# cvxopt/smcp

Measured on AMD Instinct MI355X. Metric: Newton KKT solves/sec, higher is better.
Workload: dtype f64; 1 GPU; synth50k nested block-arrow SDP n=50000, 8073 cliques, m=100; kktsolver=chol, n=50000, cliques=8073, m=100, blkval_doubles=2493568, update_doubles=10689536, parallelism=single

## Files before the change

### smcp_amd/build.py

```python
import os
import shutil
import subprocess
import sys

HERE = os.path.dirname(os.path.abspath(__file__))
CSRC = os.path.join(HERE, "csrc")
LIB = os.path.join(HERE, "libsmcp_amd.so")
SOURCES = ["capi.hip", "symbolic.cpp"]
DEPS = ["front_large.hip", "front_mfma.hip", "capi.hip", "kkt.hip", "kkt_qr.hip", "front_generic.hip", "front_mrc.hip", "front_edm.hip", "front_psd.hip", "front_downfam.hip", "front_upfam.hip", "wgblas.hpp", "context.hpp", "symbolic.cpp",
        "symbolic.hpp", "../../include/smcp_amd.h"]


def _stale():
    if not os.path.exists(LIB):
        return True
    t = os.path.getmtime(LIB)
    for d in os.listdir(CSRC):
        if os.path.getmtime(os.path.join(CSRC, d)) > t:
            return True
    return os.path.getmtime(os.path.join(HERE, "..", "include", "smcp_amd.h")) > t


def build(force=False, verbose=True):
    if not force and not _stale():
        return LIB
    hipcc = shutil.which("hipcc") or "/opt/rocm/bin/hipcc"
    cmd = [hipcc, "--offload-arch=gfx950", "-O3", "-std=c++17", "-fPIC", "-shared",
           "-Wno-unused-result", "-Wno-unused-value", "-pthread", "-o", LIB] + [os.path.join(CSRC, s) for s in SOURCES]
    if os.environ.get("SMCP_STAMPS") == "1":
        cmd.insert(1, "-DSMCP_STAMPS")
    for flag in os.environ.get("SMCP_CXXFLAGS", "").split():
        cmd.insert(1, flag)
    if verbose:
        print(" ".join(cmd), file=sys.stderr)
    subprocess.check_call(cmd)
    return LIB


if __name__ == "__main__":
    build(force="--force" in sys.argv)
```

### smcp_amd/csrc/capi.hip

```cpp
#include <hip/hip_runtime.h>
#include <memory>
#include <unordered_map>

#include <algorithm>
#include <chrono>
#include <cstdio>
#include <cstring>
#include <map>
#include <new>
#include <atomic>
#include <thread>
#include <type_traits>
#include <vector>

#include "../../include/smcp_amd.h"
#include "context.hpp"
#include "switches.hpp"
#include "front_generic.hip"
#include "front_mfma.hip"
#include "front_large.hip"
#include "front_inv.hip"
#include "front_n16.hip"
#include "front_downfam.hip"
#include "front_fam.hip"
#include "front_upfam.hip"
#include "front_fam2.hip"
#include "front_lfsp.hip"
#include "front_leafgram.hip"
#include "front_famt.hip"
#include "front_flow.hip"
#include "front_mrc.hip"
#include "front_edm.hip"
#include "front_psd.hip"

using namespace smcp;

#define HIPCHK(x)                                                                        \
  do {                                                                                   \
    hipError_t e_ = (x);                                                                 \
    if (e_ != hipSuccess) {                                                              \
      fprintf(stderr, "smcp_amd: HIP error %s at %s:%d\n", hipGetErrorString(e_), __FILE__, __LINE__); \
      return SMCP_EHIP;                                                                  \
    }                                                                                    \
  } while (0)

namespace {

enum {
  KID_chol_level = 0, KID_llt_level, KID_pinv_level, KID_gather_level, KID_completion_all,
  KID_hess_up_level, KID_hess_down_level, KID_hess_down_inv_all, KID_hess_up_inv_level, KID_scale_an,
  KID_factor_yaa, KID_trsm_fwd_level, KID_trsm_bwd_level, KID_amap, KID_aadj, KID_scatter_constraints,
  KID_dense_potrf, KID_dense_potrs, KID_vec_axpby, KID_axpby, KID_reduce_cliques, KID_reduce_final,
  KID_hess_up_mfma, KID_hess_down_mfma, KID_chol_mfma, KID_pinv_mfma, KID_prep_lk,
  KID_hess_up_mfma_hbm, KID_hess_down_mfma_hbm, KID_chol_mfma_hbm, KID_pinv_mfma_hbm,
  KID_gram_partial, KID_gram_reduce, KID_hess_up_pad,
  KID_lf_assemble, KID_lf_clear_upd, KID_lf_up1, KID_lf_up2, KID_lf_up3, KID_lf_down1, KID_lf_down2, KID_lf_down3,
  KID_lf_pinv1, KID_lf_pinv2, KID_lf_diag, KID_lf_chol_panel, KID_lf_chol_trail, KID_lf_pack_upd,
  KID_lf_prep_s, KID_lf_prep_row, KID_lf_prep_k, KID_factor_yaa_lds,
  KID_factor_inverse, KID_hess_down_inv_mfma, KID_hess_down_inv_mfma_hbm, KID_hess_up_inv_mfma, KID_hess_up_inv_mfma_hbm,
  KID_completion_mfma, KID_completion_mfma_hbm, KID_lf_copy_an, KID_lf_ri_an, KID_lf_dinv1, KID_lf_dinv2,
  KID_lf_uinv1, KID_lf_uinv2, KID_lf_completion, KID_hess_up_n16, KID_llt_mfma, KID_llt_mfma_hbm, KID_lf_llt,
  KID_hess_up_fam, KID_qr_rmul, KID_qr_dots, KID_qr_comb, KID_qr_small, KID_fam2_prep, KID_mid_chol, KID_lf_diag_inv, KID_lfsp_up, KID_lfsp_prep, KID_leaf_gram, KID_leaf_tables, KID_fam_sparse, KID_gram_diag128, KID_lf_assemble_lds, KID_fam_terms, KID_famt_prep, KID_lf_assemble_lds_dyn, KID_lf_zsp, KID_fam_terms_grp, KID_lf_assemble_fz, KID_factor_inverse_lds, KID_chol_flow,
  KID_mrc_diag, KID_mrc_rank, KID_mrc_reduce, KID_mrc_factor, KID_cut_signs, KID_cut_weights,
  KID_edm_rank, KID_edm_reduce, KID_edm_factor, KID_edm_dense, KID_hess_down_fam, KID_hess_up_fam1,
  KID_psd_zero, KID_psd_scatter, KID_psd_solve, KID_psd_fill,
  KID_COUNT
};
const char* const KID_NAMES[KID_COUNT] = {
  "k_chol_level", "k_llt_level", "k_pinv_level", "k_gather_level", "k_completion_all",
  "k_hess_up_level", "k_hess_down_level", "k_hess_down_inv_all", "k_hess_up_inv_level", "k_scale_an",
  "k_factor_yaa", "k_trsm_fwd_level", "k_trsm_bwd_level", "k_amap", "k_aadj", "k_scatter_constraints",
  "k_dense_potrf", "k_dense_potrs", "k_vec_axpby", "k_axpby", "k_reduce_cliques", "k_reduce_final",
  "k_hess_up_mfma<true>", "k_hess_down_mfma<true>", "k_chol_mfma<true>", "k_pinv_mfma<true>", "k_prep_lk",
  "k_hess_up_mfma<false>", "k_hess_down_mfma<false>", "k_chol_mfma<false>", "k_pinv_mfma<false>",
  "k_gram_partial", "k_gram_reduce", "k_hess_up_pad",
  "k_lf_assemble", "k_lf_clear_upd", "k_lf_up1", "k_lf_up2", "k_lf_up3", "k_lf_down1", "k_lf_down2", "k_lf_down3",
  "k_lf_pinv1", "k_lf_pinv2", "k_lf_diag", "k_lf_chol_panel", "k_lf_chol_trail", "k_lf_pack_upd",
  "k_lf_prep_s", "k_lf_prep_row", "k_lf_prep_k", "k_factor_yaa_lds",
  "k_factor_inverse", "k_hess_down_inv_mfma<true>", "k_hess_down_inv_mfma<false>", "k_hess_up_inv_mfma<true>",
  "k_hess_up_inv_mfma<false>", "k_completion_mfma<true>", "k_completion_mfma<false>", "k_lf_copy_an", "k_lf_ri_an",
  "k_lf_dinv1", "k_lf_dinv2", "k_lf_uinv1", "k_lf_uinv2", "k_lf_completion", "k_hess_up_n16",
  "k_llt_mfma<true>", "k_llt_mfma<false>", "k_lf_llt", "k_hess_up_fam",
  "k_stack_trsm", "k_stack_dots", "k_stack_comb", "k_qr_small", "k_fam2_prep", "k_mid_chol", "k_lf_diag_inv", "k_lfsp_up", "k_lfsp_prep", "k_leaf_pairs", "k_leaf_tables", "k_fam_sparse", "k_gram_diag128", "k_lf_assemble_lds", "k_fam_terms", "k_famt_prep", "k_lf_assemble_lds_dyn", "k_lf_zsp", "k_fam_terms_grp", "k_lf_assemble_fz", "k_factor_inverse_lds", "k_chol_flow",
  "k_mrc_diag", "k_mrc_rank", "k_mrc_reduce", "k_mrc_factor", "k_cut_signs", "k_cut_weights",
  "k_edm_rank", "k_edm_reduce", "k_edm_factor", "k_edm_dense", "k_hess_down_fam", "k_hess_up_fam1",
  "k_psd_zero", "k_psd_scatter", "k_psd_solve", "k_psd_fill"};

inline void note_launch(csp_ctx* c, int kid) {
  const hipError_t e = hipGetLastError();
  if (e != hipSuccess && !c->launch_err) {
    c->launch_err = (int)e;
    fprintf(stderr, "smcp_amd: launch of %s failed: %s\n", (kid >= 0 && kid < KID_COUNT) ? KID_NAMES[kid] : "?", hipGetErrorString(e));
  }
}
inline hipError_t end_call(csp_ctx* c) {
  hipError_t e = hipGetLastError();
  if (e == hipSuccess && c->launch_err) e = c->launch_err > 0 ? (hipError_t)c->launch_err : hipErrorLaunchFailure;
  c->launch_err = 0;
  return e;
}

__global__ void k_race_spin(long long ticks) {
  const long long t0 = wall_clock64();
  for (int it = 0; it < (1 << 22) && wall_clock64() - t0 < ticks; ++it) __builtin_amdgcn_s_sleep(8);
}
struct RaceInject {
  std::atomic<uint64_t> state{0};
  std::atomic<int64_t> injected{0};
  std::atomic<int> max_us{200};
  std::atomic<int> drop_joins{0};
  bool on() const { return state.load(std::memory_order_relaxed) != 0; }
  void seed(uint64_t s) { state.store(s ? (s * 0x9E3779B97F4A7C15ull) | 1ull : 0ull); }
  uint64_t next() {
    uint64_t x = state.load(std::memory_order_relaxed);
    x ^= x << 13; x ^= x >> 7; x ^= x << 17;
    state.store(x | 1ull, std::memory_order_relaxed);
    return x;
  }
};
// ... 592 lines not shown
    csp_ctx::FlowPlanDev P;
    P.nwg = (int)optr.size() - 1;
    int64_t junk = 0;
    if (dev_upload(&P.own_ptr, optr, junk) || dev_upload(&P.own_tile, otile, junk)) { (void)hipGetLastError(); return false; }
    c->D.bytes += junk;
    it = c->flow_plans.emplace(plan_key, P).first;
  }
  FlowArgs f;
  f.A = A; f.ld = ld; f.n = n;
  f.dinv = dinv ? dinv : W.dinv;
  f.P = W.P; f.flags = W.flags;
  f.epoch = ++W.epoch;
  f.own_ptr = it->second.own_ptr; f.own_tile = it->second.own_tile;
  f.info = info; f.info_val = info_val;
  f.cl = fa ? fa->t.cl : nullptr; f.lev = fa ? fa->t.lev : nullptr; f.mode = mode; f.nsn1 = fa ? fa->t.nsn1 : 1;
  f.dbg = nullptr;
  f.p_stride = (int64_t)ntiles * 4096; f.dinv_stride = (int64_t)nt * 4096; f.flag_stride = ntiles + nt + 4;
  static int stamps = -1;
  if (stamps < 0) stamps = sw_on("SMCP_FLOW_STAMPS", 0);
  static long long* dbg = nullptr;
  if (stamps) { if (!dbg) (void)hipMalloc((void**)&dbg, sizeof(long long) * 16 * FLOW_MAXWG); f.dbg = dbg; }
  launch_lds(c, KID_chol_flow, k_chol_flow, dim3(it->second.nwg, cnt), dim3(256), FLOW_LDS_BYTES, st, f);
  if (stamps && dbg) {
    std::vector<long long> h((size_t)8 * it->second.nwg);
    (void)hipStreamSynchronize(st);
    (void)hipMemcpy(h.data(), dbg, h.size() * sizeof(long long), hipMemcpyDeviceToHost);
    for (int w = 0; w < std::min(it->second.nwg, 20); ++w)
      fprintf(stderr, "flow n %d wg %3d: idle %7.1f us (%lld)  update %7.1f us (%lld)  potrf %7.1f us (%lld)  panel %7.1f us (%lld)\n", n, w,
              h[8 * w] / 100.0, h[8 * w + 4], h[8 * w + 1] / 100.0, h[8 * w + 5], h[8 * w + 2] / 100.0, h[8 * w + 6], h[8 * w + 3] / 100.0, h[8 * w + 7]);
  }
  return true;
}

void lf_chol(csp_ctx* c, const MfmaArgs& a, int cnt, double* x, hipStream_t st) {
  dim3 blk(256);
  const int nfmax = a.nnmax + a.namax;
  lf_assemble(c, a, cnt, 1, x, 0, 0, st, true);
  if (use_mid(nfmax)) {
    launch_lds(c, KID_mid_chol, k_mid_chol, dim3(cnt), dim3(1024), mid_chol_lds(nfmax), st, a, x, (double*)nullptr, 0);
    return;
  }
  if (cnt == 1 && a.namax == 0 && flow_chol(c, st, x, 0, a.nnmax, nullptr, &a, 0, a.t.info, 0)) return;
  const int mtA = tiles64(a.namax);
  for (int jb = 0; jb < a.nnmax; jb += LB) {
    launch_lds(c, KID_lf_diag, k_lf_diag, dim3(cnt), diag_blk(), LF_DIAG_LDS, st, a, x, (double*)nullptr, 0, jb, 1);
    const int mrem = nfmax - jb - 1, ncr = std::max(0, a.nnmax - jb - 1);
    if (mrem > 0) launch(c, KID_lf_chol_panel, k_lf_chol_panel, dim3(umax1(tiles64(mrem)), cnt), blk, st, a, x, (double*)nullptr, 0, jb);
    const int mt = tiles64(mrem), nt = tiles64(ncr);
    const int ntask = nt * (nt + 1) / 2 + std::max(0, mt - nt) * nt + mtA * (mtA + 1) / 2;
    if (ntask > 0) launch(c, KID_lf_chol_trail, k_lf_chol_trail, dim3(umax1(ntask), cnt), blk, st, a, x, (double*)nullptr, 0, jb);
  }
  if (a.namax) launch(c, KID_lf_pack_upd, k_lf_pack_upd, dim3(umax1(std::min(64, (a.namax * a.namax + 255) / 256)), cnt), blk, st, a);
}
void lf_factor_yaa(csp_ctx* c, const MfmaArgs& a, int cnt, double* fac, hipStream_t st) {
  dim3 blk(256);
  if (use_mid(a.namax)) {
    launch_lds(c, KID_mid_chol, k_mid_chol, dim3(cnt), dim3(1024), mid_chol_lds(a.namax), st, a, (double*)nullptr, fac, 2);
    return;
  }
  if (flow_chol(c, st, fac, 0, a.namax, nullptr, &a, 2, a.t.info, 0, cnt)) return;
  for (int jb = 0; jb < a.namax; jb += LB) {
    launch_lds(c, KID_lf_diag, k_lf_diag, dim3(cnt), diag_blk(), LF_DIAG_LDS, st, a, (double*)nullptr, fac, 2, jb, 1);
    const int mrem = a.namax - jb - 1;
    if (mrem > 0) {
      launch(c, KID_lf_chol_panel, k_lf_chol_panel, dim3(umax1(tiles64(mrem)), cnt), blk, st, a, (double*)nullptr, fac, 2, jb);
      const int mt = tiles64(mrem);
      launch(c, KID_lf_chol_trail, k_lf_chol_trail, dim3(umax1(mt * (mt + 1) / 2), cnt), blk, st, a, (double*)nullptr, fac, 2, jb);
    }
  }
}
void lf_prep(csp_ctx* c, const MfmaArgs& a, int cnt, const double* L, hipStream_t st) {
  dim3 blk(256);
  static int hoist = -1;
  if (hoist < 0) { const char* e = sw_str("SMCP_MID"); hoist = (e && e[0] == '0') ? 0 : 1; }
  if (hoist) {
    launch_lds(c, KID_lf_diag_inv, k_lf_diag_inv, dim3(cnt, tiles64(a.nnmax)), blk, LF_DIAG_LDS, st, a, L, c->D.lk);
    static int rec = -1;
    if (rec < 0) { const char* e = sw_str("SMCP_TRTRI"); rec = (e && e[0] == '0') ? 0 : 1; }
    if (rec) {
      for (int b = LB; b < a.nnmax; b *= 2) {
        const int pairs = (a.nnmax + 2 * b - 1) / (2 * b), tpb = b / LB;
        for (int step = 0; step < 2; ++step)
          launch(c, KID_lf_prep_s, k_lf_trtri, dim3(umax1(pairs * tpb * tpb), cnt), blk, st, a, L, c->D.lk, b, step);
      }
    } else
    for (int ib = LB; ib < a.nnmax; ib += LB) {
      launch(c, KID_lf_prep_s, k_lf_prep_s, dim3(umax1(tiles64(ib)), cnt), blk, st, a, L, c->D.lk, ib, 0);
      launch(c, KID_lf_prep_row, k_lf_prep_row, dim3(umax1(tiles64(ib)), cnt), blk, st, a, L, c->D.lk, ib, 0, 1);
    }
  } else
  for (int ib = 0; ib < a.nnmax; ib += LB) {
    launch_lds(c, KID_lf_diag, k_lf_diag, dim3(cnt), diag_blk(), LF_DIAG_LDS, st, a, const_cast<double*>(L), (double*)nullptr, 1, ib, 0);
    if (ib > 0) launch(c, KID_lf_prep_s, k_lf_prep_s, dim3(umax1(tiles64(ib)), cnt), blk, st, a, L, c->D.lk, ib, 0);
    launch(c, KID_lf_prep_row, k_lf_prep_row, dim3(umax1(tiles64(ib) + 1), cnt), blk, st, a, L, c->D.lk, ib, 0, 0);
  }
  if (a.namax) launch(c, KID_lf_prep_k, k_lf_prep_k, dim3(umax1(tiles64(a.namax) * tiles64(a.nnmax)), cnt), blk, st, a, L, c->D.lk);
}

static size_t prep_lk_lds_bytes(int nnmax) { return nnmax > 16 ? (size_t)16 * 16 * 16 * sizeof(double) : 0; }
static int prep_lk_threads(int nnmax) { return nnmax > 16 ? NT : 128; }
__global__ void k_diag_fingerprint(const CliqueDesc* cl, int nsn, const double* x, unsigned long long* slot, int* bad, int check) {
  __shared__ unsigned long long part[256];
  unsigned long long s = 0;
  for (int k = blockIdx.x; k < nsn; k += gridDim.x) {
    const CliqueDesc d = cl[k];
    const int64_t len = (int64_t)(d.nn + d.na) * d.nn;
    for (int64_t e = threadIdx.x; e < len; e += blockDim.x)
      s += (unsigned long long)__double_as_longlong(x[d.blk + e]) * (2ull * (unsigned long long)(d.blk + e) + 1ull);
  }
  part[threadIdx.x] = s;
  __syncthreads();
  for (int o = 128; o > 0; o >>= 1) { if ((int)threadIdx.x < o) part[threadIdx.x] += part[threadIdx.x + o]; __syncthreads(); }
  if (threadIdx.x == 0) atomicAdd(slot + (check ? 4 : 0), part[0]);
  (void)bad;
}
__global__ void k_fingerprint_compare(unsigned long long* slots, int which, int* bad) {
  if (threadIdx.x == 0) { if (slots[which] != slots[which + 4]) *bad = 1 + which; slots[which + 4] = 0; }
}
static void fp_record(csp_ctx* c, int which, const double* x, hipStream_t st) {
  if (!c->verify_cache || !c->D.fp) return;
  (void)hipMemsetAsync(c->D.fp + which, 0, sizeof(unsigned long long), st);
  hipLaunchKernelGGL(k_diag_fingerprint, dim3(1024), dim3(256), 0, st, c->D.cl, (int)c->S.nsn, x, c->D.fp + which, c->D.fp_bad, 0);
}
static int fp_check(csp_ctx* c, int which, const double* x, hipStream_t st) {
  if (!c->verify_cache || !c->D.fp) return 0;
  hipLaunchKernelGGL(k_diag_fingerprint, dim3(1024), dim3(256), 0, st, c->D.cl, (int)c->S.nsn, x, c->D.fp + which, c->D.fp_bad, 1);
  hipLaunchKernelGGL(k_fingerprint_compare, dim3(1), dim3(64), 0, st, c->D.fp, which, c->D.fp_bad);
  int bad = 0;
  if (hipMemcpyAsync(&bad, c->D.fp_bad, sizeof(int), hipMemcpyDeviceToHost, st) != hipSuccess || hipStreamSynchronize(st) != hipSuccess) return SMCP_EHIP;
  if (bad) {
    (void)hipMemsetAsync(c->D.fp_bad, 0, sizeof(int), st);
    fprintf(stderr, "smcp_amd: stale cache: the matrix at %p changed since the quantities cached for it (kind %d) were derived; "
                    "call csp_touch after writing to a matrix outside the library\n", (const void*)x, which);
    return SMCP_ESTALE;
  }
  return 0;
}

void prep_lk(csp_ctx* c, const double* L, hipStream_t st) {
  TreeArgs t = tree_args(c);
  if (use_large()) {
    t.lev = c->D.lev3idx;
    MfmaArgs a0 = mfma_args(c, nullptr, 0, 1);
    {
      Fork f(c, st, 0);
      for_all_large(c, a0, [&](MfmaArgs am, int cnt) { lf_prep(c, am, cnt, L, f.s); });
      if (c->D.nI_total) {
        int nnI = 0;
        for (const LevelClass& Lc : c->lvl) if (Lc.nI) nnI = std::max(nnI, (int)Lc.nnmaxI);
        launch_lds(c, KID_prep_lk, k_prep_lk, dim3((int)c->D.nI_total), dim3(prep_lk_threads(nnI)), prep_lk_lds_bytes(nnI), st, t, L, c->D.lk);
      }
    }
  } else {
    t.lev = nullptr;
    launch_lds(c, KID_prep_lk, k_prep_lk, dim3((int)c->S.nsn), dim3(NT), prep_lk_lds_bytes(1 << 20), st, t, L, c->D.lk);
  }
  c->D.lk_tag_L = L;
  c->D.lk_tag_Y = nullptr;
  c->D.part_valid = false;
  c->D.lk_gen++;
  fp_record(c, 0, L, st);
}
void prep_lk_set(csp_ctx* c, int set, const double* L, hipStream_t st) {
  TreeArgs t = tree_args(c);
  MfmaArgs a0 = mfma_args(c, nullptr, 0, 1);
  for (int64_t l = 0; l < c->S.nlev; ++l)
    for_level_classes(c, l, a0, [&](bool lds, MfmaArgs am, int cnt, size_t, int) {
      if (lds) { t.lev = am.t.lev; launch_lds(c, KID_prep_lk, k_prep_lk, dim3(cnt), dim3(prep_lk_threads(am.nnmax)), prep_lk_lds_bytes(am.nnmax), st, t, L, c->D.lk); }
      else lf_prep(c, am, cnt, L, st);
    }, set);
  c->D.lk_gen++;
}
int prep_lk_cached(csp_ctx* c, const double* L, const double* Y, hipStream_t st) {
  const bool nocache = cache_off();
  if (!nocache && c->D.lk_tag_L && c->D.lk_tag_L == L) return fp_check(c, 0, L, st);
  if (!nocache && c->D.lk_tag_Y && c->D.lk_tag_Y == Y) return fp_check(c, 1, Y, st);
  prep_lk(c, L, st);
  return 0;
}
// ... 1512 lines not shown
    if ((rc = dev_upload(&D.tmpptr, c->h_tmpptr, D.bytes))) return rc;
    if ((rc = dev_alloc(&D.yaa, S.updlen(), D.bytes))) return rc;
    if ((rc = dev_alloc(&D.fac, S.updlen(), D.bytes))) return rc;
    HIPCHK(hipMemset(D.fac, 0, sizeof(double) * std::max<int64_t>(S.updlen(), 1)));
    if (!D.sw) {
      if ((rc = dev_alloc(&D.sw, S.blklen(), D.bytes))) return rc;
      hipLaunchKernelGGL(k_fill_sqrt_weights, dim3((unsigned)std::min<int64_t>(S.nsn, 4096)), dim3(256), 0, 0, D.cl, (int)S.nsn, D.sw);
    }
    if ((rc = dev_alloc(&D.faci, S.updlen(), D.bytes))) return rc;
    if ((rc = dev_alloc(&D.red, 4096, D.bytes))) return rc;
    if ((rc = dev_alloc(&D.info, 32, D.bytes))) return rc;
    HIPCHK(hipMemset(D.info, 0, sizeof(int) * 32));
    HIPCHK(hipHostMalloc((void**)&D.info_host, 128));
    clk.mark("attributes + buffers");
    { hipDeviceProp_t p; D.ncu = (hipGetDeviceProperties(&p, device) == hipSuccess && p.multiProcessorCount > 0) ? p.multiProcessorCount : 256; }
    D.device = device;
  } else {
    if (D.upd) { hipFree(D.upd); D.bytes -= D.max_rhs * S.updlen() * 8; D.upd = nullptr; }
    if (D.updp) { hipFree(D.updp); D.bytes -= D.max_rhs * D.updp_stride * 8; D.updp = nullptr; }
    if (D.tmp) { hipFree(D.tmp); D.bytes -= D.max_rhs * D.tmplen * 8; D.tmp = nullptr; }
  }
  int rc = 0;
  if ((rc = dev_alloc(&D.upd, max_rhs * S.updlen(), D.bytes))) return rc;
  { const char* e = sw_str("SMCP_UPDP_PAD"); D.updp_stride = S.updplen() + (e ? std::max(0, atoi(e)) : 0); }
  if ((rc = dev_alloc(&D.updp, max_rhs * D.updp_stride, D.bytes))) return rc;
  if ((rc = dev_alloc(&D.tmp, max_rhs * D.tmplen, D.bytes))) return rc;
  D.max_rhs = max_rhs;
  clk.mark("per-rhs workspaces");
  return 0;
}

int64_t csp_device_bytes(const csp_ctx* c) { return c ? c->D.bytes : 0; }

static int cholesky_impl(csp_ctx* c, double* x, void* stream, int set);
int csp_cholesky(csp_ctx* c, double* x, void* stream) { return cholesky_impl(c, x, stream, 0); }
int csp_cholesky_part(csp_ctx* c, double* x, int set, void* stream) {
  if (set < 1 || set > 2 || !c || !c->sets[set].lev2 || use_generic(c)) return SMCP_EINVAL;
  return cholesky_impl(c, x, stream, set);
}
static int cholesky_impl(csp_ctx* c, double* x, void* stream, int set) {
  if (int rc = ready(c)) return rc;
  invalidate_tags(c, x);
  hipStream_t st = (hipStream_t)stream;
  TreeArgs a = tree_args(c);
  HIPCHK(zero_flag(c, st));
  if (!use_generic(c)) {
    MfmaArgs a0 = mfma_args(c, nullptr, 0, 1);
    a0.LK = nullptr;
    for (int64_t l = 0; l < c->S.nlev; ++l)
      for_level_classes(c, l, a0, [&](bool lds, MfmaArgs am, int cnt, size_t bytes, int thr) {
        if (lds) launch_lds(c, KID_chol_mfma, k_chol_mfma<true>, dim3(cnt), dim3(fact_threads(am, thr, 0)),
                            (size_t)mfma_lds_doubles_for(WK_CHOL, am.nnmax, am.namax) * sizeof(double), st, am, x, (double*)nullptr);
        else if (use_large() && c->D.gp_tptr) lf_chol(c, am, cnt, x, st);
        else launch_lds(c, KID_chol_mfma_hbm, k_chol_mfma<false>, dim3(cnt), dim3(thr), 0, st, am, x, (double*)nullptr);
      }, set);
  } else
  for_levels_up(c, [&](const int32_t* lev, int cnt) {
    a.lev = lev;
    launch(c, KID_chol_level, k_chol_level, dim3(cnt), dim3(NT), st, a, x);
  });
  HIPCHK(end_call(c));
  return fetch_info(c, st);
}

int csp_llt(csp_ctx* c, double* x, void* stream) {
  if (int rc = ready(c)) return rc;
  invalidate_tags(c, x);
  hipStream_t st = (hipStream_t)stream;
  TreeArgs a = tree_args(c);
  if (!use_generic(c)) {
    MfmaArgs a0 = mfma_args(c, nullptr, 0, 1);
    a0.LK = nullptr;
    dim3 blk(256);
    for (int64_t l = 0; l < c->S.nlev; ++l)
      for_level_classes(c, l, a0, [&](bool lds, MfmaArgs am, int cnt, size_t bytes, int thr) {
        if (lds) launch_lds(c, KID_llt_mfma, k_llt_mfma<true>, dim3(cnt), dim3(thr), bytes, st, am, x);
        else if (use_large()) {
          const int mtA = tiles64(am.namax), ntN = tiles64(am.nnmax);
          const int ntile = ntN * (ntN + 1) / 2 + mtA * ntN + mtA * (mtA + 1) / 2;
          launch(c, KID_lf_llt, k_lf_llt, dim3(umax1(ntile), cnt), blk, st, am, x, 0);
          launch(c, KID_lf_llt, k_lf_llt, dim3(umax1(ntile), cnt), blk, st, am, x, 1);
          lf_assemble(c, am, cnt, 1, x, 0, 2, st);
          if (am.namax) launch(c, KID_lf_pack_upd, k_lf_pack_upd, dim3(umax1(std::min(64, (am.namax * am.namax + 255) / 256)), cnt), blk, st, am);
        } else launch_lds(c, KID_llt_mfma_hbm, k_llt_mfma<false>, dim3(cnt), dim3(thr), 0, st, am, x);
      });
  } else
  for_levels_up(c, [&](const int32_t* lev, int cnt) {
    a.lev = lev;
    launch(c, KID_llt_level, k_llt_level, dim3(cnt), dim3(NT), st, a, x);
  });
  HIPCHK(end_call(c));
  return 0;
}

static int projected_inverse_impl(csp_ctx* c, double* x, void* stream, int set);
int csp_projected_inverse(csp_ctx* c, double* x, void* stream) { return projected_inverse_impl(c, x, stream, 0); }
int csp_projected_inverse_part(csp_ctx* c, double* x, int set, void* stream) {
  if (set < 1 || set > 2 || !c || !c->sets[set].lev2 || use_generic(c)) return SMCP_EINVAL;
  return projected_inverse_impl(c, x, stream, set);
}
static int projected_inverse_impl(csp_ctx* c, double* x, void* stream, int set) {
  if (int rc = ready(c)) return rc;
  invalidate_tags(c, x);
  hipStream_t st = (hipStream_t)stream;
  TreeArgs a = tree_args(c);
  if (!use_generic(c)) {
    if (set) { prep_lk_set(c, set, x, st); c->D.lk_tag_L = nullptr; c->D.lk_tag_Y = nullptr; }
    else {
    prep_lk(c, x, st);
    c->D.lk_tag_L = nullptr;
    c->D.lk_tag_Y = x;
    }
    const bool whole = !set;
    MfmaArgs a0 = mfma_args(c, nullptr, 0, 1);
    const bool keep_yaa = !set && !cache_off() && c->D.yaa && c->S.updlen() > 0;
    if (keep_yaa) a0.t.upd = c->D.yaa;
    for (int64_t l = c->S.nlev - 1; l >= 0; --l)
      for_level_classes(c, l, a0, [&](bool lds, MfmaArgs am, int cnt, size_t bytes, int thr) {
        if (lds) launch_lds(c, KID_pinv_mfma, k_pinv_mfma<true>, dim3(cnt), dim3(fact_threads(am, thr, 1)),
                            (size_t)mfma_lds_doubles_for(WK_PINV, am.nnmax, am.namax) * sizeof(double), st, am, x);
        else if (use_large()) lf_pinv(c, am, cnt, x, st);
        else launch_lds(c, KID_pinv_mfma_hbm, k_pinv_mfma<false>, dim3(cnt), dim3(thr), 0, st, am, x);
      }, set);
    if (keep_yaa) {
      c->D.yaa_tag = x;
      c->D.fac_tag = c->D.faci_tag = nullptr;
      c->D.part_valid = false;
      fp_record(c, 2, x, st);
    }
    if (whole) fp_record(c, 1, x, st);
  } else
  for_levels_down(c, [&](const int32_t* lev, int cnt) {
    a.lev = lev;
    launch(c, KID_pinv_level, k_pinv_level, dim3(cnt), dim3(NT), st, a, x);
  });
  HIPCHK(end_call(c));
  return 0;
}

constexpr int SCALING_FAC = 1;
static bool leafgram_ok(csp_ctx* c, int64_t mcols);
static bool scaling_overlap_on() {
  static int on = -1;
  if (on < 0) { const char* e = sw_str("SMCP_SCALING_OVERLAP"); on = (e && e[0] == '0') ? 0 : 1; }
  return on == 1;
}
static int scaling_impl(csp_ctx* c, double* L, double* Y, int flags, hipStream_t st) {
  DeviceCtx& D = c->D;
  const Symbolic& S = c->S;
  const int64_t bl = S.blklen();
  if (c->scal_lstar < 0) {
    int64_t ls = S.nlev;
    while (ls > 0 && c->lvl[(size_t)ls - 1].nI == 0) --ls;
    c->scal_lstar = ls;
    std::vector<int> lev_of((size_t)S.nsn, 0);
    for (int64_t l = 0; l < S.nlev; ++l)
      for (int64_t q = S.levptr[l]; q < S.levptr[l + 1]; ++q) lev_of[(size_t)S.levidx[q]] = (int)l;
    int64_t t0 = bl;
    for (int64_t k = 0; k < S.nsn; ++k) if (lev_of[(size_t)k] == S.nlev - 1) t0 = std::min<int64_t>(t0, S.blkptr[k]);
    for (int64_t k = 0; k < S.nsn; ++k) if (S.blkptr[k] >= t0 && lev_of[(size_t)k] != S.nlev - 1) { t0 = 0; break; }
    c->scal_tail0 = t0;
  }
  const int64_t lstar = c->scal_lstar;
  const bool fast = !use_generic(c) && use_large() && D.gp_tptr && !cache_off() && Fork::enabled() && scaling_overlap_on() &&
                    c->ntrial == 1 && lstar < S.nlev && (lstar > 0 || D.nI_total == 0) && D.yaa && S.updlen() > 0 && !c->verify_cache;
  if (!fast) {
    if (int rc = cholesky_impl(c, L, (void*)st, 0)) return rc;
    HIPCHK(hipMemcpyAsync(Y, L, sizeof(double) * bl, hipMemcpyDeviceToDevice, st));
    if (int rc = projected_inverse_impl(c, Y, (void*)st, 0)) return rc;
    c->D.lk_tag_L = L;
    if (flags & SCALING_FAC) { if (int rc = prepare_yaa(c, Y, true, st)) return rc; HIPCHK(end_call(c)); }
    return 0;
  }
  invalidate_tags(c, L);
  invalidate_tags(c, Y);
  HIPCHK(zero_flag(c, st));
  const int64_t last = S.nlev - 1;
  const int64_t tail0 = c->scal_tail0;
  MfmaArgs a0 = mfma_args(c, nullptr, 0, 1);
  a0.LK = nullptr;
  TreeArgs t = tree_args(c);
  int nnI = 0;
  for (const LevelClass& Lc : c->lvl) if (Lc.nI) nnI = std::max(nnI, (int)Lc.nnmaxI);
  static int cprep = -1;
  if (cprep < 0) { const char* e = sw_str("SMCP_CHOL_PREP"); cprep = (e && e[0] == '0') ? 0 : 1; }
  const bool fuse_prep = cprep && nnI <= 16;
  auto chol_level = [&](int64_t l) {
    for_level_classes(c, l, a0, [&](bool lds, MfmaArgs am, int cnt, size_t bytes, int thr) {
      (void)bytes;
      const size_t lb = (size_t)mfma_lds_doubles_for(WK_CHOL, am.nnmax, am.namax) * sizeof(double);
      if (lds && fuse_prep) launch_lds(c, KID_chol_mfma, k_chol_mfma<true, true>, dim3(cnt), dim3(fact_threads(am, thr, 0)), lb, st, am, L, D.lk);
      else if (lds) launch_lds(c, KID_chol_mfma, k_chol_mfma<true>, dim3(cnt), dim3(fact_threads(am, thr, 0)), lb, st, am, L, (double*)nullptr);
      else lf_chol(c, am, cnt, L, st);
    });
  };
  for (int64_t l = 0; l < last; ++l) chol_level(l);
  std::unique_ptr<Fork> f0;
  if (last > 0) f0.reset(new Fork(c, st, 1));
  hipStream_t s0 = f0 ? f0->s : st;
  chol_level(last);
  if (D.nI_total && !fuse_prep) {
    TreeArgs ts = t;
    ts.lev = D.lev3idx;
    launch_lds(c, KID_prep_lk, k_prep_lk, dim3((int)D.nI_total), dim3(prep_lk_threads(nnI)), prep_lk_lds_bytes(nnI), s0, ts, (const double*)L, D.lk);
  }
  for (int64_t ll = 0; ll < last; ++ll)
    for_level_classes(c, ll, a0, [&](bool lds, MfmaArgs am, int cnt, size_t, int) { if (!lds) lf_prep(c, am, cnt, L, s0); });
  if (tail0 > 0) (void)hipMemcpyAsync(Y, L, sizeof(double) * tail0, hipMemcpyDeviceToDevice, s0);
  for_level_classes(c, last, a0, [&](bool lds, MfmaArgs am, int cnt, size_t, int) { if (!lds) lf_prep(c, am, cnt, L, st); });
  (void)hipMemcpyAsync(Y + tail0, L + tail0, sizeof(double) * (bl - tail0), hipMemcpyDeviceToDevice, st);
  if (f0) f0->join();
  D.lk_gen++;
  D.part_valid = false;
  MfmaArgs ap = mfma_args(c, nullptr, 0, 1);
  ap.t.upd = D.yaa;
  MfmaArgs af = mfma_args(c, nullptr, 0, 1);
  const bool want_fac = (flags & SCALING_FAC) != 0;
  static int skipenv = -1;
  if (skipenv < 0) { const char* e = sw_str("SMCP_FAC_PARTIAL"); skipenv = (e && e[0] == '0') ? 0 : 1; }
  const bool skip_children = want_fac && skipenv && D.m > 0 && !D.ns && leafgram_ok(c, D.m) && c->leafgram_policy != 0;
  bool skipped = false;
  auto factor_level = [&](int64_t l, hipStream_t lds_stream, hipStream_t large_stream) {
    for_level_classes(c, l, af, [&](bool lds, MfmaArgs am, int cnt, size_t, int) {
      if (!am.namax) return;
      if (lds) {
        if (l == 0 && skip_children && am.nS > 0) { cnt -= am.nS; skipped = true; if (!cnt) return; }
        const size_t bytes = ((size_t)padld(am.namax) * am.namax + 256 + 8) * sizeof(double);
        launch_lds(c, KID_factor_yaa_lds, k_factor_yaa_lds, dim3(cnt), dim3(fact_threads(am, 256, 2)), bytes, lds_stream, am, (const double*)D.yaa, D.fac);
      } else {
        launch(c, KID_axpby, k_copy_upd_blocks, dim3(cnt, umax1(std::min(64, (am.namax * am.namax + 1023) / 1024))), dim3(256), large_stream,
               am.t, (const double*)D.yaa, D.fac);
        lf_factor_yaa(c, am, cnt, D.fac, large_stream);
      }
    });
  };
  auto pinv_level = [&](int64_t l) {
    for_level_classes(c, l, ap, [&](bool lds, MfmaArgs am, int cnt, size_t bytes, int thr) {
      (void)bytes;
      if (lds) launch_lds(c, KID_pinv_mfma, k_pinv_mfma<true>, dim3(cnt), dim3(fact_threads(am, thr, 1)),
                          (size_t)mfma_lds_doubles_for(WK_PINV, am.nnmax, am.namax) * sizeof(double), st, am, Y);
      else lf_pinv(c, am, cnt, Y, st);
    });
// ... 793 lines not shown
```

### smcp_amd/csrc/switches.hpp

```cpp
#pragma once
#include <cstdio>
#include <cstdlib>
#include <cstring>
#include <string>

extern char** environ;

namespace smcp {

struct Switch { const char* name; const char* dflt; const char* doc; };

static const Switch SWITCHES[] = {
  {"SMCP_GENERIC", "0", "1: any-size fixed-order kernels of front_generic.hip for every tree operation (as CSP_TUNE_DETERMINISTIC)"},
  {"SMCP_LARGE", "1", "0: no tiled large-front kernels (fronts beyond LDS take the one-workgroup HBM kernels)"},
  {"SMCP_NOCACHE", "0", "1: nothing derived from (L, Y) is reused between calls"},
  {"SMCP_FORK", "1", "0: no side streams, everything on the caller's stream"},
  {"SMCP_AUX_PRIO", "1", "0: side stream 0 (few-workgroup chains) at default instead of highest priority"},
  {"SMCP_AUX_PRIO1", "1", "0: side stream 1 (filler work) at default instead of lowest priority"},
  {"SMCP_EVENT_SYSFENCE", "0", "1: internal events with the default system-scope release (12 us per hand-over instead of 7)"},
  {"SMCP_SCALING_OVERLAP", "1", "0: csp_cholesky_projected_inverse as its three steps one after the other"},
  {"SMCP_CHOL_PREP", "1", "0: k_prep_lk in a launch of its own instead of inside k_chol_mfma (narrow supernodes)"},
  {"SMCP_FAC_PARTIAL", "1", "0: chol(Y_AA) of the family children always formed by the fused scaling point"},
  {"SMCP_MID", "1", "0: per-step kernels instead of k_mid_chol / k_lf_diag_inv for fronts of at most 272 rows"},
  {"SMCP_TRTRI", "1", "0: block-row triangular inversion of large fronts instead of recursive doubling"},
  {"SMCP_N16", "1", "0: no shape-specialised k_hess_up_n16"},
  {"SMCP_OLDLDS", "0", "1: k_hess_up_mfma<true> instead of the padded / n16 kernels"},
  {"SMCP_DOWN_W", "1", "0: k_hess_down_mfma instead of the one-wave k_hess_down_w"},
  {"SMCP_DOWN_FAM", "1", "most right-hand sides of a root -> leaves sweep that take the one-launch family kernel k_hess_down_fam (0: never; the per-level k_hess_down_w launches)"},
  {"SMCP_UP_FAM", "1", "most dense right-hand sides of a leaves -> root sweep that take the resident family kernel k_hess_up_fam1, the level-0 cliques outside the families riding along (0: never; k_hess_up_fam and a launch of their own for those cliques)"},
  {"SMCP_FAM", "1", "0: no family kernels (per-level sweeps with the update exchange through HBM)"},
  {"SMCP_FAM2", "1", "0: no sparse-input family kernels (k_fam_sparse, k_fam_terms): k_hess_up_fam"},
  {"SMCP_FAMT", "1", "0: no entry-driven family sweep k_fam_terms (k_fam_sparse instead)"},
  {"SMCP_FZ", "1", "0: the family parents' packed updates go through HBM (k_fam_terms writes, the extend-add reads) instead of being formed by k_lf_assemble_fz"},
  {"SMCP_FAMT_GROUP", "1", "0: no sibling groups of family parents (k_fam_terms_grp)"},
  {"SMCP_LFSP", "1", "0: dense phases instead of the sparse-input sweep k_lfsp_up of childless large fronts"},
  {"SMCP_LFSP_GROUP", "1", "0: no sibling groups in k_lfsp_up"},
  {"SMCP_ZSP", "1", "0: dense first phase of wide childless fronts instead of k_lf_zsp"},
  {"SMCP_LEAFGRAM", "1", "0: never the closed-form Gram blocks of the family children (k_leaf_tables / k_leaf_pairs)"},
  {"SMCP_LG_SIDE", "1", "0: leaf Gram blocks after the sweep on the caller's stream instead of beside the top phases"},
  {"SMCP_GRAM_EARLY", "0", "1: the Gram chunks of the levels 0 / 1 rows on the side branch beside the top fronts' phase kernels (measured slower: 3.37 against 3.22 ms per step)"},
  {"SMCP_LG_EARLY", "1", "0: leaf Gram blocks beside the phase kernels of the top fronts instead of from the start of the sweep"},
  {"SMCP_FACI_LDS", "1", "0: inverse Y_AA factors of the small fronts by block rows against HBM (k_factor_inverse) instead of in LDS"},
  {"SMCP_FZ_TAIL", "1", "0: every (front, right-hand side) pair of the fused extend-add is one workgroup's task, also in a thin last round"},
  {"SMCP_GRAM", "1", "0: reference (two-sweep) formulation of the Schur complement instead of the Gram formulation"},
  {"SMCP_SCM", "1", "0: column-sparse constraints swept like the others (no SCMcolumn2 route)"},
  {"SMCP_TRSM_MM", "1", "0: csp_trsm through the generic level kernels instead of tile products"},
  {"SMCP_ALDS", "1", "0: extend-add of large fronts by gather plan only (no LDS streaming kernel)"},
  {"SMCP_ALDS_DYN", "1", "0: one workgroup per (front, right-hand side) instead of the task-drawing grid"},
  {"SMCP_ALDS_FILL", "1", "0: k_panel_fill builds the input panels instead of the extend-add (sgn 3)"},
  {"SMCP_ASM", "plan", "t: tiled extend-add kernel instead of the gather plan"},
  {"SMCP_ROOT_FUSED", "0", "1: fused two-product sweep of fronts without separator (Y_NN explicit: condition squared; studies only)"},
  {"SMCP_PD", "0", "1: four-wave tile products everywhere (no sixteen-wave shape for small launches)"},
  {"SMCP_POTRF_OLD", "0", "1: generic one-workgroup dense Cholesky"},
  {"SMCP_FLOW", "1", "0: no one-launch blocked Cholesky with in-launch tile dataflow (front_flow.hip): per-step kernels for dense matrices / single fronts beyond 272 rows"},
  {"SMCP_FLOW_WG", "112", "workgroups of that launch (at most 112: four launches fit the chip side by side)"},
  {"SMCP_POTRS_OLD", "0", "1: generic one-workgroup dense solve"},
// ... 69 lines not shown
```

Baseline: 337.9 KKT solves/s.

## Add register-resident fused top-front Cholesky with inverse for fronts up to 208 rows

Adds k_top_chol, a one-workgroup kernel that keeps the front's tiles in MFMA registers across waves while one wave factors and inverts the 16x16 diagonal blocks. Optionally, in the same launch, it forms the inverse of L (LK) that lf_prep would otherwise build with k_lf_diag_inv/k_lf_trtri. It is used for large-front levels of at most 208 rows in place of k_mid_chol, and the scaling-point path skips the separate inverse-preparation launches when the fused kernel already produced them. The aim is fewer launches and less LDS/HBM traffic for the top fronts, at the cost of heavy register use and more complex cache-tag invalidation.

After: 342.5 KKT solves/s, median of 6. 1.01x the previous value.

```diff
diff --git a/smcp_amd/build.py b/smcp_amd/build.py
--- a/smcp_amd/build.py
+++ b/smcp_amd/build.py
@@ -7,7 +7,7 @@
 CSRC = os.path.join(HERE, "csrc")
 LIB = os.path.join(HERE, "libsmcp_amd.so")
 SOURCES = ["capi.hip", "symbolic.cpp"]
-DEPS = ["front_large.hip", "front_mfma.hip", "capi.hip", "kkt.hip", "kkt_qr.hip", "front_generic.hip", "front_mrc.hip", "front_edm.hip", "front_psd.hip", "front_downfam.hip", "front_upfam.hip", "wgblas.hpp", "context.hpp", "symbolic.cpp",
+DEPS = ["front_large.hip", "front_top.hip", "front_mfma.hip", "capi.hip", "kkt.hip", "kkt_qr.hip", "front_generic.hip", "front_mrc.hip", "front_edm.hip", "front_psd.hip", "front_downfam.hip", "front_upfam.hip", "wgblas.hpp", "context.hpp", "symbolic.cpp",
         "symbolic.hpp", "../../include/smcp_amd.h"]
 
 
diff --git a/smcp_amd/csrc/capi.hip b/smcp_amd/csrc/capi.hip
--- a/smcp_amd/csrc/capi.hip
+++ b/smcp_amd/csrc/capi.hip
@@ -19,6 +19,7 @@
 #include "front_generic.hip"
 #include "front_mfma.hip"
 #include "front_large.hip"
+#include "front_top.hip"
 #include "front_inv.hip"
 #include "front_n16.hip"
 #include "front_downfam.hip"
@@ -63,7 +64,7 @@
   KID_hess_up_fam, KID_qr_rmul, KID_qr_dots, KID_qr_comb, KID_qr_small, KID_fam2_prep, KID_mid_chol, KID_lf_diag_inv, KID_lfsp_up, KID_lfsp_prep, KID_leaf_gram, KID_leaf_tables, KID_fam_sparse, KID_gram_diag128, KID_lf_assemble_lds, KID_fam_terms, KID_famt_prep, KID_lf_assemble_lds_dyn, KID_lf_zsp, KID_fam_terms_grp, KID_lf_assemble_fz, KID_factor_inverse_lds, KID_chol_flow,
   KID_mrc_diag, KID_mrc_rank, KID_mrc_reduce, KID_mrc_factor, KID_cut_signs, KID_cut_weights,
   KID_edm_rank, KID_edm_reduce, KID_edm_factor, KID_edm_dense, KID_hess_down_fam, KID_hess_up_fam1,
-  KID_psd_zero, KID_psd_scatter, KID_psd_solve, KID_psd_fill,
+  KID_psd_zero, KID_psd_scatter, KID_psd_solve, KID_psd_fill, KID_top_chol, KID_lf_trtri,
   KID_COUNT
 };
 const char* const KID_NAMES[KID_COUNT] = {
@@ -84,7 +85,7 @@
   "k_stack_trsm", "k_stack_dots", "k_stack_comb", "k_qr_small", "k_fam2_prep", "k_mid_chol", "k_lf_diag_inv", "k_lfsp_up", "k_lfsp_prep", "k_leaf_pairs", "k_leaf_tables", "k_fam_sparse", "k_gram_diag128", "k_lf_assemble_lds", "k_fam_terms", "k_famt_prep", "k_lf_assemble_lds_dyn", "k_lf_zsp", "k_fam_terms_grp", "k_lf_assemble_fz", "k_factor_inverse_lds", "k_chol_flow",
   "k_mrc_diag", "k_mrc_rank", "k_mrc_reduce", "k_mrc_factor", "k_cut_signs", "k_cut_weights",
   "k_edm_rank", "k_edm_reduce", "k_edm_factor", "k_edm_dense", "k_hess_down_fam", "k_hess_up_fam1",
-  "k_psd_zero", "k_psd_scatter", "k_psd_solve", "k_psd_fill"};
+  "k_psd_zero", "k_psd_scatter", "k_psd_solve", "k_psd_fill", "k_top_chol", "k_lf_trtri"};
 
 inline void note_launch(csp_ctx* c, int kid) {
   const hipError_t e = hipGetLastError();
@@ -743,10 +744,20 @@
   return true;
 }
 
-void lf_chol(csp_ctx* c, const MfmaArgs& a, int cnt, double* x, hipStream_t st) {
+bool use_top(int rowsmax) {
+  static int g = -1;
+  if (g < 0) g = sw_on("SMCP_TOP_FUSED", 1);
+  return g == 1 && rowsmax <= TOP_MAXROWS && use_mid(rowsmax);
+}
+void lf_chol(csp_ctx* c, const MfmaArgs& a, int cnt, double* x, hipStream_t st, bool with_li = false) {
   dim3 blk(256);
   const int nfmax = a.nnmax + a.namax;
   lf_assemble(c, a, cnt, 1, x, 0, 0, st, true);
+  if (use_top(nfmax)) {
+    if (with_li) launch(c, KID_top_chol, k_top_chol<true>, dim3(cnt), dim3(1024), st, a, x, c->D.lk);
+    else launch(c, KID_top_chol, k_top_chol<false>, dim3(cnt), dim3(1024), st, a, x, (double*)nullptr);
+    return;
+  }
   if (use_mid(nfmax)) {
     launch_lds(c, KID_mid_chol, k_mid_chol, dim3(cnt), dim3(1024), mid_chol_lds(nfmax), st, a, x, (double*)nullptr, 0);
     return;
@@ -780,11 +791,12 @@
     }
   }
 }
-void lf_prep(csp_ctx* c, const MfmaArgs& a, int cnt, const double* L, hipStream_t st) {
+void lf_prep(csp_ctx* c, const MfmaArgs& a, int cnt, const double* L, hipStream_t st, bool have_li = false) {
   dim3 blk(256);
   static int hoist = -1;
   if (hoist < 0) { const char* e = sw_str("SMCP_MID"); hoist = (e && e[0] == '0') ? 0 : 1; }
-  if (hoist) {
+  if (have_li) {
+  } else if (hoist) {
     launch_lds(c, KID_lf_diag_inv, k_lf_diag_inv, dim3(cnt, tiles64(a.nnmax)), blk, LF_DIAG_LDS, st, a, L, c->D.lk);
     static int rec = -1;
     if (rec < 0) { const char* e = sw_str("SMCP_TRTRI"); rec = (e && e[0] == '0') ? 0 : 1; }
@@ -792,7 +804,7 @@
       for (int b = LB; b < a.nnmax; b *= 2) {
         const int pairs = (a.nnmax + 2 * b - 1) / (2 * b), tpb = b / LB;
         for (int step = 0; step < 2; ++step)
-          launch(c, KID_lf_prep_s, k_lf_trtri, dim3(umax1(pairs * tpb * tpb), cnt), blk, st, a, L, c->D.lk, b, step);
+          launch(c, KID_lf_trtri, k_lf_trtri, dim3(umax1(pairs * tpb * tpb), cnt), blk, st, a, L, c->D.lk, b, step);
       }
     } else
     for (int ib = LB; ib < a.nnmax; ib += LB) {
@@ -848,14 +860,19 @@
   return 0;
 }
 
-void prep_lk(csp_ctx* c, const double* L, hipStream_t st) {
+static bool top_li_whole(csp_ctx* c) {
+  if (use_generic(c) || !use_large() || !c->D.gp_tptr || !c->D.nII_total || c->lvl.empty()) return false;
+  const LevelClass& Lc = c->lvl.back();
+  return c->D.nII_total == Lc.nII && use_top(Lc.nnmaxII + Lc.namaxII);
+}
+void prep_lk(csp_ctx* c, const double* L, hipStream_t st, bool have_li = false) {
   TreeArgs t = tree_args(c);
   if (use_large()) {
     t.lev = c->D.lev3idx;
     MfmaArgs a0 = mfma_args(c, nullptr, 0, 1);
     {
       Fork f(c, st, 0);
-      for_all_large(c, a0, [&](MfmaArgs am, int cnt) { lf_prep(c, am, cnt, L, f.s); });
+      for_all_large(c, a0, [&](MfmaArgs am, int cnt) { lf_prep(c, am, cnt, L, f.s, have_li); });
       if (c->D.nI_total) {
         int nnI = 0;
         for (const LevelClass& Lc : c->lvl) if (Lc.nI) nnI = std::max(nnI, (int)Lc.nnmaxI);
@@ -2434,13 +2451,13 @@
 
 int64_t csp_device_bytes(const csp_ctx* c) { return c ? c->D.bytes : 0; }
 
-static int cholesky_impl(csp_ctx* c, double* x, void* stream, int set);
+static int cholesky_impl(csp_ctx* c, double* x, void* stream, int set, bool li_last = false);
 int csp_cholesky(csp_ctx* c, double* x, void* stream) { return cholesky_impl(c, x, stream, 0); }
 int csp_cholesky_part(csp_ctx* c, double* x, int set, void* stream) {
   if (set < 1 || set > 2 || !c || !c->sets[set].lev2 || use_generic(c)) return SMCP_EINVAL;
   return cholesky_impl(c, x, stream, set);
 }
-static int cholesky_impl(csp_ctx* c, double* x, void* stream, int set) {
+static int cholesky_impl(csp_ctx* c, double* x, void* stream, int set, bool li_last) {
   if (int rc = ready(c)) return rc;
   invalidate_tags(c, x);
   hipStream_t st = (hipStream_t)stream;
@@ -2453,7 +2470,7 @@
       for_level_classes(c, l, a0, [&](bool lds, MfmaArgs am, int cnt, size_t bytes, int thr) {
         if (lds) launch_lds(c, KID_chol_mfma, k_chol_mfma<true>, dim3(cnt), dim3(fact_threads(am, thr, 0)),
                             (size_t)mfma_lds_doubles_for(WK_CHOL, am.nnmax, am.namax) * sizeof(double), st, am, x, (double*)nullptr);
-        else if (use_large() && c->D.gp_tptr) lf_chol(c, am, cnt, x, st);
+        else if (use_large() && c->D.gp_tptr) lf_chol(c, am, cnt, x, st, li_last && l == c->S.nlev - 1);
         else launch_lds(c, KID_chol_mfma_hbm, k_chol_mfma<false>, dim3(cnt), dim3(thr), 0, st, am, x, (double*)nullptr);
       }, set);
   } else
@@ -2495,13 +2512,13 @@
   return 0;
 }
 
-static int projected_inverse_impl(csp_ctx* c, double* x, void* stream, int set);
+static int projected_inverse_impl(csp_ctx* c, double* x, void* stream, int set, bool have_li = false);
 int csp_projected_inverse(csp_ctx* c, double* x, void* stream) { return projected_inverse_impl(c, x, stream, 0); }
 int csp_projected_inverse_part(csp_ctx* c, double* x, int set, void* stream) {
   if (set < 1 || set > 2 || !c || !c->sets[set].lev2 || use_generic(c)) return SMCP_EINVAL;
   return projected_inverse_impl(c, x, stream, set);
 }
-static int projected_inverse_impl(csp_ctx* c, double* x, void* stream, int set) {
+static int projected_inverse_impl(csp_ctx* c, double* x, void* stream, int set, bool have_li) {
   if (int rc = ready(c)) return rc;
   invalidate_tags(c, x);
   hipStream_t st = (hipStream_t)stream;
@@ -2509,7 +2526,7 @@
   if (!use_generic(c)) {
     if (set) { prep_lk_set(c, set, x, st); c->D.lk_tag_L = nullptr; c->D.lk_tag_Y = nullptr; }
     else {
-    prep_lk(c, x, st);
+    prep_lk(c, x, st, have_li);
     c->D.lk_tag_L = nullptr;
     c->D.lk_tag_Y = x;
     }
@@ -2567,9 +2584,11 @@
   const bool fast = !use_generic(c) && use_large() && D.gp_tptr && !cache_off() && Fork::enabled() && scaling_overlap_on() &&
                     c->ntrial == 1 && lstar < S.nlev && (lstar > 0 || D.nI_total == 0) && D.yaa && S.updlen() > 0 && !c->verify_cache;
   if (!fast) {
-    if (int rc = cholesky_impl(c, L, (void*)st, 0)) return rc;
+    const bool li = top_li_whole(c);
+    if (li) { D.lk_tag_L = D.lk_tag_Y = nullptr; D.part_valid = false; D.lk_gen++; }
+    if (int rc = cholesky_impl(c, L, (void*)st, 0, li)) return rc;
     HIPCHK(hipMemcpyAsync(Y, L, sizeof(double) * bl, hipMemcpyDeviceToDevice, st));
-    if (int rc = projected_inverse_impl(c, Y, (void*)st, 0)) return rc;
+    if (int rc = projected_inverse_impl(c, Y, (void*)st, 0, li)) return rc;
     c->D.lk_tag_L = L;
     if (flags & SCALING_FAC) { if (int rc = prepare_yaa(c, Y, true, st)) return rc; HIPCHK(end_call(c)); }
     return 0;
@@ -2593,7 +2612,7 @@
       const size_t lb = (size_t)mfma_lds_doubles_for(WK_CHOL, am.nnmax, am.namax) * sizeof(double);
       if (lds && fuse_prep) launch_lds(c, KID_chol_mfma, k_chol_mfma<true, true>, dim3(cnt), dim3(fact_threads(am, thr, 0)), lb, st, am, L, D.lk);
       else if (lds) launch_lds(c, KID_chol_mfma, k_chol_mfma<true>, dim3(cnt), dim3(fact_threads(am, thr, 0)), lb, st, am, L, (double*)nullptr);
-      else lf_chol(c, am, cnt, L, st);
+      else lf_chol(c, am, cnt, L, st, l == last);
     });
   };
   for (int64_t l = 0; l < last; ++l) chol_level(l);
@@ -2609,7 +2628,7 @@
   for (int64_t ll = 0; ll < last; ++ll)
     for_level_classes(c, ll, a0, [&](bool lds, MfmaArgs am, int cnt, size_t, int) { if (!lds) lf_prep(c, am, cnt, L, s0); });
   if (tail0 > 0) (void)hipMemcpyAsync(Y, L, sizeof(double) * tail0, hipMemcpyDeviceToDevice, s0);
-  for_level_classes(c, last, a0, [&](bool lds, MfmaArgs am, int cnt, size_t, int) { if (!lds) lf_prep(c, am, cnt, L, st); });
+  for_level_classes(c, last, a0, [&](bool lds, MfmaArgs am, int cnt, size_t, int) { if (!lds) lf_prep(c, am, cnt, L, st, use_top(am.nnmax + am.namax)); });
   (void)hipMemcpyAsync(Y + tail0, L + tail0, sizeof(double) * (bl - tail0), hipMemcpyDeviceToDevice, st);
   if (f0) f0->join();
   D.lk_gen++;
diff --git a/smcp_amd/csrc/front_top.hip b/smcp_amd/csrc/front_top.hip
--- /dev/null
+++ b/smcp_amd/csrc/front_top.hip
@@ -0,0 +1,198 @@
+#pragma once
+
+namespace smcp {
+
+constexpr int TOP_MAXT = 13;
+constexpr int TOP_MAXROWS = 16 * TOP_MAXT;
+constexpr int TOP_TW = 15;
+constexpr int TOP_SLOTS = (TOP_MAXT * (TOP_MAXT + 1) / 2 + TOP_TW - 1) / TOP_TW;
+
+#define TOP_WAVE_FENCE() do { __builtin_amdgcn_fence(__ATOMIC_RELEASE, "wavefront"); __builtin_amdgcn_wave_barrier(); \
+                              __builtin_amdgcn_fence(__ATOMIC_ACQUIRE, "wavefront"); } while (0)
+
+template <bool INV>
+__global__ void __launch_bounds__(1024) k_top_chol(MfmaArgs a, double* x, double* LK) {
+  __shared__ __attribute__((aligned(16))) double s_d[256];
+  __shared__ __attribute__((aligned(16))) double s_inv[TOP_MAXT * 256];
+  __shared__ __attribute__((aligned(16))) double s_pan[TOP_MAXT * 256];
+  __shared__ int s_fail;
+  const int k = a.t.lev[blockIdx.x];
+  if (*info_of(a.t, k)) return;
+  const CliqueDesc d = a.t.cl[k];
+  const int nn = d.nn, na = d.na, nf = nn + na;
+  if (nf > TOP_MAXROWS) return;
+  const int tid = threadIdx.x, lane = tid & 63, wave = __builtin_amdgcn_readfirstlane(tid >> 6), l15 = lane & 15, kq = lane >> 4;
+  const int nt = (nf + 15) >> 4, nct = (nn + 15) >> 4, ntile = nt * (nt + 1) / 2;
+  double* const P = x + d.blk;
+  if (tid == 0) s_fail = 0;
+  __syncthreads();
+
+  if (wave == TOP_TW) {
+    for (int r = 0; r < nct; ++r) {
+      __syncthreads();
+      const bool ok = wave_potrf_inv16(s_d, 16, min(16, nn - 16 * r), s_inv + 256 * r);
+      if (!ok && lane == 0) s_fail = 1;
+      __syncthreads();
+      if (!ok) { if (lane == 0) atomicCAS(info_of(a.t, k), 0, info_val(a.t, k)); return; }
+      __syncthreads();
+    }
+  } else {
+    const double* const U = a.t.upd + d.upd;
+    unsigned vo[4], vu[4];
+#pragma unroll
+    for (int q = 0; q < 4; ++q) { vo[q] = l15 + (kq + 4 * q) * nf; vu[q] = l15 + (kq + 4 * q) * na; }
+    int ti[TOP_SLOTS], tj[TOP_SLOTS];
+    bool valid[TOP_SLOTS];
+    d4 T[TOP_SLOTS];
+#pragma unroll
+    for (int s = 0; s < TOP_SLOTS; ++s) {
+      const int t = TOP_TW * s + wave;
+      int i = 0;
+      while ((i + 1) * (i + 2) / 2 <= t) ++i;
+      ti[s] = i; tj[s] = t - i * (i + 1) / 2;
+      valid[s] = t < ntile;
+#pragma unroll
+      for (int q = 0; q < 4; ++q) {
+        const int row = 16 * i + l15, col = 16 * tj[s] + kq + 4 * q;
+        const bool ok = valid[s] && row < nf && col <= row;
+        const double* src = !ok ? P : (col < nn ? &(P + (16 * i + 16 * tj[s] * nf))[vo[q]] : &(U + ((16 * i - nn) + (16 * tj[s] - nn) * na))[vu[q]]);
+        const double v = *src;
+        T[s][q] = ok ? v : 0.0;
+      }
+      __builtin_amdgcn_sched_barrier(0);
+    }
+    auto update = [&](d4& t, int i, int j) {
+      const double* Pi = s_pan + 256 * i;
+      const double* Pj = s_pan + 256 * j;
+#pragma unroll
+      for (int q = 0; q < 4; ++q) t = __builtin_amdgcn_mfma_f64_16x16x4f64(Pj[l15 + 16 * (4 * q + kq)], -Pi[l15 + 16 * (4 * q + kq)], t, 0, 0, 0);
+      __builtin_amdgcn_sched_barrier(0);
+    };
+    for (int r = 0; r < nct; ++r) {
+      const int bw = min(16, nn - 16 * r);
+      const bool part = bw < 16;
+#pragma unroll
+      for (int s = 0; s < TOP_SLOTS; ++s)
+        if (valid[s] && ti[s] == r && tj[s] == r) {
+          if (r > 0) update(T[s], r, r);
+#pragma unroll
+          for (int q = 0; q < 4; ++q) s_d[l15 + 16 * (kq + 4 * q)] = T[s][q];
+        }
+      __syncthreads();
+      if (r > 0) {
+#pragma unroll
+        for (int s = 0; s < TOP_SLOTS; ++s)
+          if (valid[s] && tj[s] >= r && ti[s] > r) update(T[s], ti[s], tj[s]);
+      }
+      __syncthreads();
+      if (s_fail) return;
+      int l15b = l15, kqb = kq;
+      asm volatile("" : "+v"(l15b), "+v"(kqb));
+      const double* Xr = s_inv + 256 * r;
+#pragma unroll
+      for (int s = 0; s < TOP_SLOTS; ++s) {
+        if (!valid[s] || tj[s] != r) continue;
+        const bool diag = ti[s] == r;
+        if (diag) {
+#pragma unroll
+          for (int q = 0; q < 4; ++q) {
+            const int col = kqb + 4 * q;
+            if (l15b < bw && col <= l15b) {
+              T[s][q] = s_d[l15b + 16 * col];
+              (P + (16 * r + 16 * r * nf))[vo[q]] = T[s][q];
+            }
+          }
+          if (!part) continue;
+        }
+        d4 p = {0.0, 0.0, 0.0, 0.0};
+#pragma unroll
+        for (int q = 0; q < 4; ++q) {
+          const double av = (!part || 4 * q + kqb < bw) ? T[s][q] : 0.0;
+          p = __builtin_amdgcn_mfma_f64_16x16x4f64(Xr[l15b + 16 * (4 * q + kqb)], av, p, 0, 0, 0);
+        }
+        double* Ps = s_pan + 256 * ti[s];
+        const int row = 16 * ti[s] + l15b;
+        const bool below = !diag || l15b >= bw;
+#pragma unroll
+        for (int q = 0; q < 4; ++q) {
+          const int col = kqb + 4 * q;
+          const double v = below ? p[q] : 0.0;
+          Ps[l15b + 16 * col] = v;
+          if (below && col < bw) {
+            T[s][q] = v;
+            if (row < nf) (P + (16 * ti[s] + 16 * r * nf))[vo[q]] = v;
+          }
+        }
+        __builtin_amdgcn_sched_barrier(0);
+      }
+      __syncthreads();
+    }
+    if (na > 0) {
+      const int j0 = (nn & 15) ? nct - 1 : nct;
+      double* UP = a.t.updp + d.updp;
+      int l15f = l15, kqf = kq;
+      asm volatile("" : "+v"(l15f), "+v"(kqf));
+#pragma unroll
+      for (int s = 0; s < TOP_SLOTS; ++s) {
+        if (!valid[s] || tj[s] < j0) continue;
+        update(T[s], ti[s], tj[s]);
+#pragma unroll
+        for (int q = 0; q < 4; ++q) {
+          const int row = 16 * ti[s] + l15f, col = 16 * tj[s] + kqf + 4 * q;
+          if (row < nf && col >= nn && col <= row) UP[pk_idx(row - nn, col - nn, na)] = T[s][q];
+        }
+      }
+    }
+  }
+  if (!INV) return;
+  for (int c = wave; c < nct; c += 16) {
+    const int cw = min(16, nn - 16 * c);
+    double* Xc = LK + d.blk + (int64_t)(16 * c) * nf;
+    const bool mok = l15 < cw;
+    for (int e = lane; e < 16 * c * cw; e += 64) Xc[e % (16 * c) + (int64_t)(e / (16 * c)) * nf] = 0.0;
+    d4 z;
+#pragma unroll
+    for (int q = 0; q < 4; ++q) {
+      const int n = kq + 4 * q;
+      z[q] = n >= l15 ? s_inv[256 * c + n + 16 * l15] : 0.0;
+      if (mok && n < cw) Xc[(16 * c + n) + (int64_t)l15 * nf] = z[q];
+    }
+    const double* __restrict__ Lp = P;
+    double* __restrict__ Xw = Xc;
+    const bool lastok = 16 * (nct - 1) + l15 < nn;
+    const unsigned lo = l15 + kq * nf, lo_last = (lastok ? l15 : 0) + kq * nf;
+    d4 S[TOP_MAXT - 1];
+#pragma unroll
+    for (int j = 0; j < TOP_MAXT - 1; ++j) S[j] = d4{0.0, 0.0, 0.0, 0.0};
+#pragma unroll
+    for (int ks = 0; ks < TOP_MAXT - 1; ++ks) {
+      const int kt = c + ks;
+      if (kt + 1 < nct) {
+#pragma unroll
+        for (int j = ks; j < TOP_MAXT - 1; ++j) {
+          const int r = min(c + 1 + j, nct - 1);
+          const bool last = r == nct - 1;
+          const bool rok = c + 1 + j < nct && (!last || lastok);
+#pragma unroll
+          for (int q = 0; q < 4; ++q) {
+            const double b0 = (Lp + (16 * r + (16 * kt + 4 * q) * nf))[last ? lo_last : lo];
+            S[j] = __builtin_amdgcn_mfma_f64_16x16x4f64(rok ? b0 : 0.0, z[q], S[j], 0, 0, 0);
+          }
+        }
+        const int r = kt + 1, rw = min(16, nn - 16 * r);
+        d4 zn = {0.0, 0.0, 0.0, 0.0};
+#pragma unroll
+        for (int q = 0; q < 4; ++q) zn = __builtin_amdgcn_mfma_f64_16x16x4f64(s_inv[256 * r + l15 + 16 * (4 * q + kq)], S[ks][q], zn, 0, 0, 0);
+#pragma unroll
+        for (int q = 0; q < 4; ++q) {
+          const int n = kq + 4 * q;
+          z[q] = -zn[q];
+          if (mok && n < rw) Xw[(16 * r + n) + (int64_t)l15 * nf] = z[q];
+        }
+      }
+    }
+  }
+}
+#undef TOP_WAVE_FENCE
+
+}
diff --git a/smcp_amd/csrc/switches.hpp b/smcp_amd/csrc/switches.hpp
--- a/smcp_amd/csrc/switches.hpp
+++ b/smcp_amd/csrc/switches.hpp
@@ -22,6 +22,7 @@
   {"SMCP_CHOL_PREP", "1", "0: k_prep_lk in a launch of its own instead of inside k_chol_mfma (narrow supernodes)"},
   {"SMCP_FAC_PARTIAL", "1", "0: chol(Y_AA) of the family children always formed by the fused scaling point"},
   {"SMCP_MID", "1", "0: per-step kernels instead of k_mid_chol / k_lf_diag_inv for fronts of at most 272 rows"},
+  {"SMCP_TOP_FUSED", "1", "0: k_mid_chol, and k_lf_diag_inv / k_lf_trtri for the inverse at the scaling point, instead of the register-resident k_top_chol for fronts of at most 208 rows"},
   {"SMCP_TRTRI", "1", "0: block-row triangular inversion of large fronts instead of recursive doubling"},
   {"SMCP_N16", "1", "0: no shape-specialised k_hess_up_n16"},
   {"SMCP_OLDLDS", "0", "1: k_hess_up_mfma<true> instead of the padded / n16 kernels"},
```
